# drowe67/radae

Hardware: AMD Instinct MI355X
Metric: vocoder-feature frames/sec (enc+chan+dec), model19 (higher is better)
Workload: dtype f32 I/O, 2xf16 (22-bit) MFMA operands, f32 accumulate (refine: f64 MFMA)

## Files before the change

### radae_amd/csrc/rade_core_step.hip

```cpp
#include <hip/hip_runtime.h>
#include <stdint.h>
#include <math.h>

#include "rade_devutil.h"

#define CS_THREADS 512
#define CS_WAVES (CS_THREADS / 64)
#define CS_PS 320
#define CS_WMAX 864

template <typename T> __device__ __forceinline__ T cs_gload(const T *p) { return *(const __attribute__((address_space(1))) T *)p; }

struct CsShared {
    __attribute__((aligned(16))) float x[CS_WMAX];
    __attribute__((aligned(16))) float hist[2][CS_WMAX];
    __attribute__((aligned(16))) float vin[96];
    __attribute__((aligned(16))) float h[5][96];
    __attribute__((aligned(16))) float hc[96];
    __attribute__((aligned(16))) float gh[288];
    __attribute__((aligned(16))) float pa[CS_WAVES][CS_PS];
    __attribute__((aligned(16))) float pb[CS_WAVES][CS_PS];
};

struct Rows3 { const float *r[3]; };
__device__ __forceinline__ const float *cs_in(const float *v, int) { return v; }
__device__ __forceinline__ const float *cs_in(const Rows3 &v, int q) { return v.r[q]; }
template <class T> __device__ __forceinline__ T *cs_prow(T (*part)[CS_PS], int w, int) { return part[w]; }
template <class T> __device__ __forceinline__ T *cs_prow(T (*part)[3][CS_PS], int w, int q) { return part[w][q]; }
template <int R> __device__ __forceinline__ int cs_wave()
{
    if constexpr (R == 3) return __builtin_amdgcn_readfirstlane((int)(threadIdx.x >> 6)); else return threadIdx.x >> 6;
}

template <int NRB, int NCI> struct WQ { f16x8 w[NRB][NCI]; };
template <int NRB, int NCI, int I0 = 0, int I1 = NCI>
__device__ __forceinline__ void cs_issue(const rd_mv &L, WQ<NRB, NCI> &r)
{
    const int lane = threadIdx.x & 63, wave = threadIdx.x >> 6, nch = L.K >> 3;
#pragma unroll
    for (int i = I0; i < I1; i++) {
        const int c = min(wave + CS_WAVES * i, nch - 1);
#pragma unroll
        for (int rb = 0; rb < NRB; rb++) r.w[rb][i] = cs_gload((const f16x8 *)(L.wq + ((size_t)c * (NRB * 64) + rb * 64 + lane) * 8));
    }
}
template <int NRB, int NCI>
__device__ __forceinline__ void cs_consume(const rd_mv &L, const WQ<NRB, NCI> &r, const float *v0, int K0, const float *v1, float (*part)[CS_PS])
{
    const int lane = threadIdx.x & 63, wave = threadIdx.x >> 6, nch = L.K >> 3;
    float acc[NRB];
#pragma unroll
    for (int rb = 0; rb < NRB; rb++) acc[rb] = 0.0f;
#pragma unroll
    for (int i = 0; i < NCI; i++) {
        const int c = wave + CS_WAVES * i, k = 8 * min(c, nch - 1);
        const float *src = k < K0 ? v0 + k : v1 + (k - K0);
        f32x4 a = *(const f32x4 *)src, b = *(const f32x4 *)(src + 4);
// ... 275 lines not shown
    cs_issue<2, CCI, C2, CCI>(a.conv[l], cq);
    if (!LAST) cs_issue<3, 1>(a.ghh[l + 1], hn);
    __builtin_amdgcn_sched_barrier(0);
    cs_acc3_range<2, CCI, C1, C2>(a.conv[l], cq, t0, cin, xr, cacc);
    __builtin_amdgcn_sched_barrier(0);
    cs_acc3_range<2, CCI, C2, CCI>(a.conv[l], cq, t0, cin, xr, cacc);
    cs_store3<2>(cacc, sh->pa);
    if (!LAST) cs_consume<3, 1>(a.ghh[l + 1], hn, sh->h[l + 1], H, sh->h[l + 1], sh->pb);
    __builtin_amdgcn_sched_barrier(0);
    if (!LAST) cs_issue<3, GNEXT, 0, (GNEXT < 6 ? GNEXT : 6)>(a.gin[l + 1], gnext);
    __syncthreads();
    if (tid < 96) {
#pragma unroll
        for (int q = 0; q < 3; q++) sh->x[q][cin + tid] = clamp1(tanhf(cs_row(a.conv[l], sh->pa, tid, q)));
    } else if (!LAST && tid >= 128 && tid < 128 + 3 * H) sh->gh[tid - 128] = cs_row(a.ghh[l + 1], sh->pb, tid - 128);
    __syncthreads();
}

__global__ __launch_bounds__(CS_THREADS) void k_tx_frame3(const rd_core_args *ap, unsigned seq)
{
    extern __shared__ __attribute__((aligned(16))) unsigned char cs_raw[];
    CsShared3 *sh = (CsShared3 *)cs_raw;
    const rd_core_args &a = *ap;
    const int tid = threadIdx.x, W = 864, H = 64;
    WQ<3, 1> g0, h0;
    cs_issue<3, 1>(a.gin[0], g0); cs_issue<3, 1>(a.ghh[0], h0);
    for (int i = tid; i < 2 * W; i += CS_THREADS) sh->hist[i / W][i % W] = a.hist[i];
    if (tid < 5 * H) sh->h[tid / H][tid % H] = a.h[tid];
    if (tid < 3 * 96) { const int q = tid / 96, c = tid % 96; sh->vin[q][c] = c < a.n_in ? a.in[q * a.n_in + c] : 0.0f; }
    __syncthreads();
    const Rows3 vr = { { sh->vin[0], sh->vin[1], sh->vin[2] } };
    cs_f32_product<2, 3>(a.dense1, 1, vr, sh->pa);
    cs_consume<3, 1>(a.ghh[0], h0, sh->h[0], H, sh->h[0], sh->pb);
    __syncthreads();
    if (tid < 64) {
#pragma unroll
        for (int q = 0; q < 3; q++) sh->x[q][tid] = clamp1(tanhf(cs_row(a.dense1, sh->pa, tid, q)));
    } else if (tid >= 128 && tid < 128 + 3 * H) sh->gh[tid - 128] = cs_row(a.ghh[0], sh->pb, tid - 128);
    __syncthreads();
    WQ<3, 4> g1; WQ<3, 6> g2; WQ<3, 9> g3; WQ<3, 11> g4;
    cs_enc_layer3<1, 4, 4, false>(sh, a, 0, 64, g0, g1);
    cs_enc_layer3<4, 9, 6, false>(sh, a, 1, 224, g1, g2);
    cs_enc_layer3<6, 14, 9, false>(sh, a, 2, 384, g2, g3);
    cs_enc_layer3<9, 19, 11, false>(sh, a, 3, 544, g3, g4);
    cs_enc_layer3<11, 24, 11, true>(sh, a, 4, 704, g4, g4);
    const Rows3 xr = { { sh->x[0], sh->x[1], sh->x[2] } };
    cs_f32_product<14, 3>(a.out, 2, xr, sh->pa);
    for (int i = tid; i < W; i += CS_THREADS) { a.hist[i] = sh->x[2][i]; a.hist[W + i] = sh->x[1][i]; }
    if (tid < 5 * H) a.h[tid] = sh->h[tid / H][tid % H];
    __syncthreads();
    if (tid < 3 * RD_LATENT) { const int q = tid / RD_LATENT, c = tid % RD_LATENT; sh->zs[q * RD_LATENT + c] = cs_row(a.out, sh->pa, c, q); }
    __syncthreads();
    const float *zs = sh->zs;
    const rd_tables *tab = ap->tab;
    float2 *out = (float2 *)ap->iq_out;
    if (tid < RD_M) {
        f32x2 acc[RD_NS + 1];
#pragma unroll
        for (int s = 0; s <= RD_NS; s++) acc[s] = (f32x2){ 0.0f, 0.0f };
#pragma unroll 6
        for (int c = 0; c < RD_NC; c++) {
            const float2 w = ld2(tab->Winv[c], tid);
            acc[0] = idft_term(acc[0], make_float2(tab->P[c] * tab->pilot_gain, 0.0f * tab->pilot_gain), w);
#pragma unroll
            for (int s = 1; s <= RD_NS; s++) { const int k = (s - 1) * RD_NC + c; acc[s] = idft_term(acc[s], make_float2(zs[2 * k], zs[2 * k + 1]), w); }
        }
#pragma unroll
        for (int s = 0; s <= RD_NS; s++) {
            const float2 v = pa_limit(make_float2(acc[s][0], acc[s][1]));
            out[s * RD_SYM + RD_NCP + tid] = v;
            if (tid >= RD_M - RD_NCP) out[s * RD_SYM + tid - (RD_M - RD_NCP)] = v;
        }
        __threadfence_system();
    }
    __syncthreads();
    if (tid == 0 && ap->done) { __threadfence_system(); *(volatile unsigned *)ap->done = seq; }
}
extern "C" int rd_launch_tx_frame(const rd_core_args *a_dev, unsigned seq, rd_stream_t s)
{
    rd_dyn_lds_once<k_tx_frame3, (int)sizeof(CsShared3)>();
    hipLaunchKernelGGL(k_tx_frame3, dim3(1), dim3(CS_THREADS), sizeof(CsShared3), (hipStream_t)s, a_dev, seq);
    return (int)hipGetLastError();
}

extern "C" int rd_launch_core_step(const rd_core_args *a, rd_stream_t s)
{
    if (a->is_enc) rd_dyn_lds_once<k_core_enc_step, (int)sizeof(CsShared)>(); else rd_dyn_lds_once<k_core_dec_step, (int)sizeof(CsShared)>();
    if (a->is_enc) hipLaunchKernelGGL(k_core_enc_step, dim3(1), dim3(CS_THREADS), sizeof(CsShared), (hipStream_t)s, *a);
    else hipLaunchKernelGGL(k_core_dec_step, dim3(1), dim3(CS_THREADS), sizeof(CsShared), (hipStream_t)s, *a);
    return (int)hipGetLastError();
}
```

### radae_amd/csrc/rade_dev.h

```cpp
#ifndef RADE_DEV_H
#define RADE_DEV_H

#include <stdint.h>

#ifdef __cplusplus
extern "C" {
#endif

#define RD_M        160
#define RD_NCP      32
#define RD_SYM      192
#define RD_NC       30
#define RD_NS       4
#define RD_NMF      960
#define RD_NEOO     1152
#define RD_RXBUF    2112
#define RD_NFC      40
#define RD_NQ       16
#define RD_NTAP     101
#define RD_NINMAX   1120
#define RD_LATENT   80
#define RD_ZMF      240
#define RD_FEAT_MF  432
#define RD_NEOOBITS 180
#define RD_ENC_W    864
#define RD_DEC_W    736
#define RD_ENC_IN   96
#define RD_RX_ROUND_MAX 128
#define RD_DEC_ROWS_MAX (3 * RD_RX_ROUND_MAX)

typedef struct {
    float Winv[RD_NC][RD_M][2];
    float Wfwd[RD_M][RD_NC][2];
    float P[RD_NC], Pend[RD_NC];
    float p[RD_M][2], pend[RD_M][2];
    float eoo[RD_NEOO][2];
    float Pmat[RD_NC][2][3][2];
    float eq_rot[RD_NC][2];
    float bpf_h[RD_NTAP + 3];
    float bpf_E[RD_NEOO][2];
    float p_w[RD_M][RD_NFC][2];
    double fcoarse[RD_NFC];
    float pilot_gain;
    float snr_c1, snr_c2;
    float pad;
} rd_tables;

typedef struct {
    int mem_len;
    int grid_off;
    float phase[2];
    float mem[102][2];
} rd_bpf_state;

typedef struct {
    int state, nin, tmax, tmax_candidate, valid_count, uw_errors, synced_count, mf;
    int f_ind_max, dec_reset_pending, n_out_frames, pad0;
    uint32_t lcg; int has_eoo, dt_valid;
    int pad1;
    double fmax, foff_err, rx_phase[2];
    double rx_theta;
    double Dthresh, Dtmax12, Dtmax12_eoo;
    float snr_est, pad2[3];
    unsigned rxmax[4];
    long long consumed;
    rd_bpf_state bpf;
    float rx_buf[RD_RXBUF][2];
    float rowsum1[RD_NMF], rowsum2[RD_NMF];
} rd_rx_stream;

typedef struct {
    int n_calls;
    int n_rows;
    int uw_from_row;
    int consumed;
    int row_reset[RD_DEC_ROWS_MAX];
    int call_ret[RD_RX_ROUND_MAX];
    int call_row_lo[RD_RX_ROUND_MAX], call_row_hi[RD_RX_ROUND_MAX];
    int call_trace_idx[RD_RX_ROUND_MAX];
    int out_base;
    int pad[3];
} rd_rx_round;

typedef struct {
    int state_before, state_after, nin_before, nin_after, ret, tmax, f_ind_max, valid_count;
    int uw_errors, synced_count, snr_int, pad;
    double fmax, Dthresh, Dtmax12, Dtmax12_eoo;
    float snrdB_3k_est; float pad2;
} rd_rx_trace;

typedef void *rd_stream_t;

typedef struct {
    const float *a1; long a1_sb, a1_st; int K1;
    const float *a0; long a0_sb, a0_st; int K0;
    const int *reset; int reset_sb;
    const int *n_rows;
    const float *Wp; const float *bias;
    const unsigned short *Wp16;
    const float *Wscale;
    float *y; long y_sb, y_st; int N;
    int B, T, act;
} rd_gemm_args;
int rd_launch_gemm(const rd_gemm_args *a, rd_stream_t s);
long rd_pack_weights(const float *W, int N, int K, float *out);
long rd_packed_size(int N, int K);

typedef struct {
    const float *gi; long gi_sb, gi_st;
    const float *Whh; const float *bhh;
    float *h;
    float *out; long out_sb, out_st;
    const int *reset; int reset_sb;
    const int *n_rows;
    int B, T, H;
    unsigned short *outf; int outf_NQ, outf_col;
} rd_scan_args;
int rd_launch_gru_scan(const rd_scan_args *a, rd_stream_t s);

#define RD_EF_KB   (RD_ENC_W / 16)
#define RD_EF_TILE (RD_EF_KB * 1024)
typedef struct {
    const unsigned short *xf; int NQ;
    int B, T, K0, K1, dil;
    const unsigned short *Wp16; const float *Wscale; const float *bias; int N, act;
    float *y; long y_sb, y_st;
    unsigned short *yf; int ycol;
    int seq_taps, no_pair;
    int pair;
    const float *xin; int Kin; const float *Wp;
} rd_encf_args;
int rd_launch_encf_gemm(const rd_encf_args *a, rd_stream_t s);
int rd_launch_encf_dense1(const rd_encf_args *a, rd_stream_t s);
int rd_launch_encf_hist(unsigned short *xf, int NQ, float *x32, long x32_sb, int B, int T, int dir, rd_stream_t s);

int rd_launch_enc_pack(const float *features, float *xin, int B, int T, rd_stream_t s);
int rd_launch_pad_rows(const float *src, float *dst, long R, int K, int Kpad, rd_stream_t s);
int rd_launch_chan_symbol(const float *z, const float *H, const float *noise, float *out, long n_real, int mode, float p0, float p1, unsigned long long seed, rd_stream_t s);
int rd_launch_carry_rows(float *x, int B, int Tcap, int W, int nhist, int T, const int *n_rows, rd_stream_t s);
int rd_launch_ofdm_mod(const rd_tables *tab, const float *z, void *tx, long tx_stride, int B, int n_mf, int linear, rd_stream_t s);
int rd_launch_ofdm_mod_mp(const rd_tables *tab, const float *z, void *tx, long tx_stride, int B, int n_mf, const void *G, void *mp, double *part, int linear, rd_stream_t s);
int rd_launch_eoo_build(const rd_tables *tab, const float *bits, float *eoo, int B, rd_stream_t s);
int rd_launch_copy_eoo(const float *eoo, void *out, long stride, int B, rd_stream_t s);

enum { RD_IRX_LS = 0, RD_IRX_MEAN6 = 1, RD_IRX_ALL = 2, RD_IRX_NONE = 3 };
typedef struct {
    const rd_tables *tab; const void *rx; long rx_stride;
    const float *foff;
    int n_mf, time_offset, eq, coarse_mag, B;
    float mag_scale;
    float *z_hat;
    double *part;
    const float *z_ref; long long *n_err;
} rd_irx_args;
int rd_launch_irx(const rd_irx_args *a, rd_stream_t s);

#define RD_LOSS_WG 64
typedef struct {
    const float *feat; long f_stride; int f_row;
    const float *hat; long h_stride; int h_row;
    const int *len;
    double *part_v; int *part_s; int n_blk;
    double *loss; int *start;
    float *frame_loss; long fl_stride; int max_hat;
    int B;
} rd_loss_args;
int rd_launch_loss(const rd_loss_args *a, rd_stream_t s);

#define RD_RS_NCH 8
typedef struct {
    const rd_tables *tab; const float *z, *H; const void *noise; float *z_hat;
    int B, n_steps, has_phase; float sigma, ph_re, ph_im;
    const float *sigma_b;
    unsigned long long seed;
    double *part;
    double *stats;
} rd_rs_args;
int rd_launch_rs_pa(const rd_rs_args *a, rd_stream_t s);

#define RD_CLK_TILE 1024
#define RD_CLK_PHASES 256
#define RD_CLK_TAPS 32
typedef struct { long long step_q, t0_q, n0, in_base; int n_in, n_out; } rd_clk_stream;
typedef struct {
    const void *x; long x_stride; void *y; long y_stride;
    const rd_clk_stream *ps;
    const float *taps;
    int mode, B, max_out;
} rd_clk_args;
int rd_launch_clk_resample(const rd_clk_args *a, rd_stream_t s);

#define RD_WIRE_NCH_MAX 64
// ... 339 lines not shown
```

### radae_amd/csrc/rade_engine.c

```c
#define _GNU_SOURCE

#include <pthread.h>
#include <time.h>
#include <sched.h>
#include <stdio.h>
#include <stdlib.h>
#include <string.h>
#include <stdint.h>
#include <math.h>

#include "rade_batch.h"
#include "rade_api.h"
#include "rade_host.h"
#include "rade_engine.h"

#define CHK(x) do { hipError_t e_ = (x); if (e_ != hipSuccess) { fprintf(stderr, "rade: HIP error %s at %s:%d\n", hipGetErrorString(e_), __FILE__, __LINE__); goto fail; } } while (0)

static int g_engines_open;
double rade_host_cpu_quota(void)
{
    cpu_set_t set; double n = 1.0;
    if (sched_getaffinity(0, sizeof set, &set) == 0) n = (double)CPU_COUNT(&set);
    FILE *f = fopen("/sys/fs/cgroup/cpu.max", "r");
    if (f) {
// ... 141 lines not shown
    }
    if (tx) {
        h->enc_hist_frag = 0;
        if (h->tx_bpf) hipMemcpyAsync(h->tx_bpf, h->tx_bpf_init, sizeof(rd_bpf_state) * h->B, hipMemcpyDeviceToDevice, st);
        r.enc_h = h->enc_h[0];
        r.enc_x = h->enc_x; r.enc_x_sb = (long)(2 + h->Tcap) * RD_ENC_W;
    }
    rd_launch_reset(&r, st);
}

void rade_batch_rx_reset(rade_batch *h) { ON_DEV(h); reset_on(h, 0, 1, NULL); hipDeviceSynchronize(); }

void rade_batch_reset(rade_batch *h, void *stream) { ON_DEV(h); reset_on(h, 1, 1, stream); }

void rade_batch_rx_set_lcg(rade_batch *h, const unsigned *seeds_host)
{
    ON_DEV(h);
    if (!h) return;
    for (int b = 0; b < h->B; b++) h->lcg_seeds[b] = seeds_host ? seeds_host[b] : 1u;
    hipMemcpy(h->d_lcg_seeds, h->lcg_seeds, sizeof(unsigned) * h->B, hipMemcpyHostToDevice);
    rade_batch_rx_reset(h);
}

void rade_batch_tx_reset(rade_batch *h) { ON_DEV(h); reset_on(h, 1, 0, NULL); hipDeviceSynchronize(); }

rade_batch *rade_batch_open_mem(const void *blob, size_t blob_len, const rade_batch_config *cfg)
{
    rade_batch *h = NULL;
    rd_model m; int have_model = 0;
    if (!cfg || cfg->n_streams <= 0 || cfg->max_tx_mf <= 0) { fprintf(stderr, "rade: bad batch config\n"); return NULL; }
    int ndev = 0;
    if (hipGetDeviceCount(&ndev) != hipSuccess || ndev <= 0) {
        fprintf(stderr, "rade: no HIP device available -- this library has no CPU fallback\n");
        return NULL;
    }
    CHK(hipSetDevice(cfg->device));
    if (rd_model_parse(blob, blob_len, &m)) return NULL;
    have_model = 1;
    h = calloc(1, sizeof *h);
    if (!h) { rd_model_free(&m); return NULL; }
    __atomic_add_fetch(&g_engines_open, 1, __ATOMIC_RELAXED);
    h->B = cfg->n_streams; h->max_tx_mf = cfg->max_tx_mf; h->device = cfg->device; h->flags = cfg->flags;
    h->trace_cap = cfg->rx_trace_calls; h->Tcap = 3 * cfg->max_tx_mf;
    h->unsync_off_after = cfg->disable_unsync != 0.0f ? (int)((double)cfg->disable_unsync * 8000.0 / RD_NMF) : -1;
    const size_t B = (size_t)h->B, T = (size_t)h->Tcap;
    h->R = getenv("RADE_ROUND_CALLS") ? atoi(getenv("RADE_ROUND_CALLS")) : RD_RX_ROUND_MAX;
    if (h->R < 1) h->R = 1;
    if (h->R > RD_RX_ROUND_MAX) h->R = RD_RX_ROUND_MAX;
    h->dec_rows = getenv("RADE_DEC_ROWS") ? atoi(getenv("RADE_DEC_ROWS")) : 48;
    if (h->dec_rows < 3) h->dec_rows = 3;
    if (h->dec_rows > 63) h->dec_rows = 63;
    const size_t DR = (size_t)h->dec_rows;

    rd_tables *tab = malloc(sizeof *tab);
    rd_tables_fill(tab);
    h->d_tab = dev_upload(h, tab, sizeof *tab);
    h->corrq16 = upload_table16(h, tab, rd_corrq16_table_fill, RD_CORRQ16_HALFS);
    h->corra16 = upload_table16(h, tab, rd_corra16_table_fill, RD_CORRA16_HALFS);
    h->wfwd16 = upload_table16(h, tab, rd_wfwd16_table_fill, RD_WFWD16_HALFS);
    h->bpf16 = upload_table16(h, tab, rd_bpf16_table_fill, RD_BPF16_HALFS);
    free(tab);
    {
        double vm[8][RD_M];
        for (int n = 0; n < RD_M; n++) { const double nu = ((double)n - 79.5) / 80.0; double v = 1.0; for (int m = 0; m < 8; m++) { vm[m][n] = v; v *= nu; } }
        h->vm = dev_upload(h, vm, sizeof vm);
    }
    h->rx_lds = rd_rx_sync_prepare();
    h->rx_census = getenv("RADE_RX2_CENSUS") ? atoi(getenv("RADE_RX2_CENSUS")) : 0;
    if (h->alloc_failed || h->rx_lds <= 0) goto fail;

    int err = 0;
    h->feat_in = m.enc_dense1.n_in; h->enc_kpad = (h->feat_in + 15) & ~15; h->bottleneck1 = (cfg->flags & RADE_BATCH_BOTTLENECK1) != 0;
    err |= upload_lin(h, &h->enc_dense1, m.enc_dense1.w, m.enc_dense1.b, NULL, 64, h->feat_in, h->enc_kpad);
    err |= upload_lin(h, &h->enc_zdense, m.enc_zdense.w, m.enc_zdense.b, NULL, 80, 864, 864);
    err |= upload_lin(h, &h->dec_dense1, m.dec_dense1.w, m.dec_dense1.b, NULL, 96, 80, 80);
    err |= upload_lin(h, &h->dec_output, m.dec_output.w, m.dec_output.b, NULL, h->feat_in, 736, 736);
    for (int l = 0; l < 5 && !err; l++) {
        err |= upload_lin(h, &h->enc_gin[l], m.enc_gru[l].w_ih, m.enc_gru[l].b_ih, m.enc_gru[l].s_ih, 192, ENC_IN[l], ENC_IN[l]);
        err |= upload_lin(h, &h->dec_gin[l], m.dec_gru[l].w_ih, m.dec_gru[l].b_ih, m.dec_gru[l].s_ih, 288, DEC_IN[l], DEC_IN[l]);
        err |= upload_lin(h, &h->enc_conv[l], m.enc_conv[l].w, m.enc_conv[l].b, m.enc_conv[l].row_scale, 96, m.enc_conv[l].n_in, m.enc_conv[l].n_in);
        err |= upload_lin(h, &h->dec_conv[l], m.dec_conv[l].w, m.dec_conv[l].b, m.dec_conv[l].row_scale, 32, m.dec_conv[l].n_in, m.dec_conv[l].n_in);
        err |= upload_lin(h, &h->dec_glu[l], m.dec_glu[l].w, NULL, m.dec_glu[l].row_scale, 96, 96, 96);
        h->enc_whh[l] = dev_upload(h, m.enc_gru[l].w_hh, sizeof(float) * 192 * 64);
        h->enc_bhh[l] = dev_upload(h, m.enc_gru[l].b_hh, sizeof(float) * 192);
        h->dec_whh[l] = dev_upload(h, m.dec_gru[l].w_hh, sizeof(float) * 288 * 96);
        h->dec_bhh[l] = dev_upload(h, m.dec_gru[l].b_hh, sizeof(float) * 288);
        if (m.dec_gru[l].s_hh) {
            unsigned short *pa = malloc(sizeof(unsigned short) * rd_packed16a_size(288, 96)); float *scl = malloc(sizeof(float) * 288);
            const long nq = (pa && scl) ? rd_pack_weights_q16_a16(m.dec_gru[l].w_hh, m.dec_gru[l].s_hh, 288, 96, pa, scl) : -1;
            if (nq > 0) { h->dec_whq[l] = dev_upload_opt(h, pa, sizeof(unsigned short) * nq); h->dec_whs[l] = dev_upload_opt(h, scl, sizeof(float) * 288); }
            free(pa); free(scl);
        }
    }
    if (err || h->alloc_failed) { fprintf(stderr, "rade: weight upload failed\n"); goto fail; }

    h->enc_xin = dev_zeros(h, sizeof(float) * B * T * RD_ENC_IN);
    h->enc_x = dev_zeros(h, sizeof(float) * B * (2 + T) * RD_ENC_W);
    h->enc_gi = dev_zeros(h, sizeof(float) * B * T * 192);
    h->enc_nq = 1 + (h->Tcap + 31) / 32;
    h->enc_seq_taps = getenv("RADE_ENCF_SEQ_TAPS") != NULL;
    h->enc_no_pair = getenv("RADE_ENCF_NO_PAIR") != NULL;
    if (B * T > 16384 && !getenv("RADE_ENC_ROWS")) {
        h->enc_xf = dev_alloc_opt(h, sizeof(unsigned short) * B * h->enc_nq * RD_EF_TILE, 1);
        if (!h->enc_xf && !getenv("RADE_VERBOSE_0"))
            fprintf(stderr, "rade: no device memory for the encoder's fragment buffer (%.1f MB): the float32-row kernels serve every call (slower encoder GEMMs, same results to the last bits documented in rade_batch.h)\n",
                    1e-6 * sizeof(unsigned short) * (double)B * h->enc_nq * RD_EF_TILE);
    }
    h->enc_z = dev_zeros(h, sizeof(float) * B * T * RD_LATENT);
    h->eoo = dev_zeros(h, sizeof(float) * B * RD_NEOO * 2);
    h->eoo_bits = dev_zeros(h, sizeof(float) * B * RD_NEOOBITS);
    h->bypass_dec = (cfg->flags & RADE_BATCH_BYPASS_DEC) != 0;
    h->tx_linear = (cfg->flags & RADE_BATCH_TX_LINEAR) != 0;
    if (h->tx_linear && (cfg->flags & RADE_BATCH_TX_BPF)) { fprintf(stderr, "rade: RADE_BATCH_TX_LINEAR cannot be combined with RADE_BATCH_TX_BPF (the filter clips)\n"); goto fail; }
    if (cfg->flags & RADE_BATCH_TX_BPF) {
// ... 679 lines not shown
```

### radae_amd/csrc/rade_host.c

```c
#include "rade_host.h"
#include "rade_batch.h"

#include <math.h>
#include <stdio.h>
#include <stdlib.h>
#include <string.h>

#define PI_D 3.14159265358979323846

static void pa_limit_host(float *re, float *im)
{
    float mag = hypotf(*re, *im), ang = atan2f(*im, *re), t = tanhf(mag);
    *re = t * cosf(ang); *im = t * sinf(ang);
}

void rd_tables_fill(rd_tables *T)
{
    static const float barker13[13] = { 1, 1, 1, 1, 1, -1, -1, 1, 1, -1, 1, -1, 1 };
    float w[RD_NC];
    memset(T, 0, sizeof *T);
    const float two_pi = (float)(2.0 * PI_D);
    for (int c = 0; c < RD_NC; c++) w[c] = (two_pi * (float)(15 + c)) / 160.0f;
    for (int c = 0; c < RD_NC; c++)
        for (int n = 0; n < RD_M; n++) {
// ... 430 lines not shown
                    o[0] = hi; o[64 * 8] = lo;
                }
}
void rd_corra16_table_fill(const rd_tables *T, unsigned short *out )
{
    static double q[RD_NQ][RD_M], alr[RD_NQ][RD_NFC], ali[RD_NQ][RD_NFC];
    corr_basis(T, q, alr, ali);
    for (int nt = 0; nt < 5; nt++)
        for (int lane = 0; lane < 64; lane++)
            for (int j = 0; j < 8; j++) {
                const int n = 16 * nt + (lane & 15), f = n >> 1, cpp = n & 1;
                const int g = lane >> 4, np_ = j < 4 ? 4 * g + j : 16 + 4 * g + (j - 4), r = np_ >> 1, cp = np_ & 1;
                const double ar = alr[r][f], ai = ali[r][f];
                const float v = (float)(1024.0 * (cpp == 0 ? (cp == 0 ? ar : -ai) : (cp == 0 ? ai : ar)));
                const unsigned short hi = f32_to_f16(v), lo = f32_to_f16(v - f16_to_f32(hi));
                unsigned short *o = out + (((size_t)nt * 2) * 64 + lane) * 8 + j;
                o[0] = hi; o[64 * 8] = lo;
            }
}
double rd_corr_tables_check(const rd_tables *T)
{
    static double q[RD_NQ][RD_M], alr[RD_NQ][RD_NFC], ali[RD_NQ][RD_NFC];
    corr_basis(T, q, alr, ali);
    double worst = 0.0;
    for (int m = 0; m < RD_M; m++)
        for (int f = 0; f < RD_NFC; f++) {
            double re = 0.0, im = 0.0;
            for (int r = 0; r < RD_NQ; r++) {
                const double sr = (double)T->p[m][0] * q[r][m], si = (double)T->p[m][1] * q[r][m];
                re += alr[r][f] * sr - ali[r][f] * si; im += alr[r][f] * si + ali[r][f] * sr;
            }
            const double d = hypot(re - (double)T->p_w[m][f][0], im - (double)T->p_w[m][f][1]);
            if (d > worst) worst = d;
        }
    return worst;
}

void rd_wfwd16_table_fill(const rd_tables *T, unsigned short *out )
{
    for (int tile = 0; tile < 2; tile++)
        for (int s = 0; s < 10; s++)
            for (int lane = 0; lane < 64; lane++)
                for (int j = 0; j < 8; j++) {
                    const int c = 16 * tile + (lane & 15);
                    const int k = 32 * s + 8 * (lane >> 4) + j, n = k >> 1, comp = k & 1;
                    float v = 0.0f;
                    if (c < RD_NC) v = 4096.0f * (comp == 0 ? T->Wfwd[n][c][0] : -T->Wfwd[n][c][1]);
                    const unsigned short hi = f32_to_f16(v), lo = f32_to_f16(v - f16_to_f32(hi));
                    unsigned short *o = out + ((((size_t)tile * 10 + s) * 2) * 64 + lane) * 8 + j;
                    o[0] = hi; o[64 * 8] = lo;
                }
}

void rd_bpf16_table_fill(const rd_tables *T, unsigned short *out )
{
    for (int ks = 0; ks < 4; ks++)
        for (int lane = 0; lane < 64; lane++)
            for (int j = 0; j < 8; j++) {
                const int r = lane & 15, m = 32 * ks + 8 * (lane >> 4) + j, t = m - r;
                const float v = (t >= 0 && t < RD_NTAP) ? 1024.0f * T->bpf_h[t] : 0.0f;
                const unsigned short hi = f32_to_f16(v), lo = f32_to_f16(v - f16_to_f32(hi));
                unsigned short *o = out + (((size_t)ks * 2) * 64 + lane) * 8 + j;
                o[0] = hi; o[64 * 8] = lo;
            }
}

static double bessel_i0(double x)
{
    double s = 1.0, t = 1.0;
    for (int k = 1; k < 40; k++) { t *= (x * 0.5) / k; s += t * t; }
    return s;
}

void rade_resample_taps(float *out )
{
    const double i0b = bessel_i0(10.0);
    for (int p = 0; p <= 256; p++) {
        const double f = p / 256.0, sf = sin(PI_D * (p <= 128 ? f : 1.0 - f));
        double g[32], sum = 0.0;
        for (int j = 0; j < 32; j++) {
            const int k = j - 15;
            const double t = (double)k - f, u = t / 16.0;
            const double sinc = t == 0.0 ? 1.0 : ((k & 1) ? sf : -sf) / (PI_D * t);
            g[j] = fabs(t) <= 16.0 ? sinc * bessel_i0(10.0 * sqrt(1.0 - u * u)) / i0b : 0.0;
            sum += g[j];
        }
        for (int j = 0; j < 32; j++) out[p * 32 + j] = (float)(g[j] / sum);
    }
}

int rd_resample_q(double t0, double ppm, long long *step_q, long long *t0_q)
{
    if (!(fabs(ppm) <= 50000.0) || !(fabs(t0) <= 536870912.0)) return -1;
    *step_q = llrint((1.0 + ppm * 1e-6) * 4294967296.0);
    *t0_q = llrint(t0 * 4294967296.0);
    return 0;
}

long long rade_resample_count(long long in_end, double t0, double ppm)
{
    long long step_q, t0_q;
    if (rd_resample_q(t0, ppm, &step_q, &t0_q)) return -1;
    const __int128 need = ((__int128)in_end << 32) - t0_q;
    if (need <= 0) return 0;
    const __int128 n = (need + step_q - 1) / step_q;
    return n * step_q > ((__int128)1 << 62) ? -1 : (long long)n;
// ... 337 lines not shown
```

### radae_amd/csrc/rade_host.h

```cpp
#ifndef RADE_HOST_H
#define RADE_HOST_H

#include <stddef.h>

#include "rade_dev.h"
#include "rade_batch.h"

#ifdef __cplusplus
extern "C" {
#endif

typedef struct { int n_in, n_out; float *w, *b; float *row_scale; } rd_linear;
typedef struct { int n_in, hid; float *w_ih, *w_hh, *b_ih, *b_hh; float *s_ih, *s_hh; } rd_gru;

typedef struct {
    rd_linear enc_dense1, enc_zdense, dec_dense1, dec_output;
    rd_gru enc_gru[5], dec_gru[5];
    rd_linear enc_conv[5], dec_conv[5];
    rd_linear dec_glu[5];
} rd_model;

const char *rd_find_default_model(const char *hint, char *buf, size_t n);

void rd_tables_fill(rd_tables *T);
int rd_model_parse(const void *blob, size_t len, rd_model *m);
void rd_model_free(rd_model *m);

long rd_packed16_size(int N, int K);
#define RD_CORRQ16_HALFS (2 * 10 * 2 * 64 * 8)
#define RD_CORRA16_HALFS (5 * 2 * 64 * 8)
#define RD_WFWD16_HALFS  (2 * 10 * 2 * 64 * 8)
#define RD_BPF16_HALFS   (4 * 2 * 64 * 8)
void rd_corrq16_table_fill(const rd_tables *T, unsigned short *out);
void rd_corra16_table_fill(const rd_tables *T, unsigned short *out);
double rd_corr_tables_check(const rd_tables *T);
void rd_wfwd16_table_fill(const rd_tables *T, unsigned short *out);
void rd_bpf16_table_fill(const rd_tables *T, unsigned short *out);
long rd_pack_weights_f16x2(const float *W, int N, int K, unsigned short *out);
long rd_pack_weights_q16(const float *W, const float *row_scale, int N, int K, unsigned short *out, float *scale_out);
int rd_chunkmajor_q16(const float *W, const float *row_scale, int N, int K, int Kpad, int Npad, unsigned short *out);
void rd_chunkmajor_f32(const float *W, int N, int K, int Kpad, int Npad, float *out);
long rd_packed16a_size(int N, int K);
long rd_pack_weights_q16_a16(const float *W, const float *row_scale, int N, int K, unsigned short *out, float *scale_out);
long rd_pack_weights_f16x2_a16(const float *W, int N, int K, unsigned short *out);
int rd_resample_q(double t0, double ppm, long long *step_q, long long *t0_q);
int rd_rate_reduce(int L, int M, int *Lr, int *Mr, int *T);
void rd_cno_table(int N, float *out);
void rd_cno_finish(const rade_cno_plan_t *q, const rade_cno_params *p, const double *bands, int n_windows, rade_cno_result *res);
#ifdef __cplusplus
}
#endif
void *rd_core_tx_open(const void *blob, int len, const rd_tables *d_tab);
void rd_core_tx_close(void *t);
int rd_core_tx_frame(void *t, const float *features_in, float *tx_out);
struct rade_batch;
const rd_tables *rd_batch_tables(const struct rade_batch *h);
int rd_batch_has_tx_bpf(const struct rade_batch *h);

#endif
```

### radae_amd/csrc/rade_kernels.hip

```cpp
#include "rade_devutil.h"

__device__ float g_zero_row[2048];

#include "rade_gemm.h"
#include "rade_gru_scan.h"
#include "rade_rows.h"
#include "rade_ofdm_mod.h"
#include "rade_chan.h"
```

### radae_amd/csrc/rade_ofdm_mod.h

```cpp
template <bool LINEAR>
__global__ __launch_bounds__(192) void k_ofdm_mod(const rd_tables *tab, const float *z, float2 *tx, long tx_stride, int n_mf)
{
    __shared__ float2 sym[RD_NS + 1][RD_NC];
    const int mf = blockIdx.x, b = blockIdx.y, tid = threadIdx.x;
    const float *zf = z + ((size_t)b * n_mf + mf) * RD_ZMF;
    const float pg = LINEAR ? 1.0f : tab->pilot_gain;
    if (tid < RD_NC) sym[0][tid] = make_float2(tab->P[tid] * pg, 0.0f * pg);
    if (tid < 120) sym[1 + tid / RD_NC][tid % RD_NC] = make_float2(zf[2 * tid], zf[2 * tid + 1]);
    __syncthreads();
    float2 *out = tx + (size_t)b * tx_stride + (size_t)mf * RD_NMF;
    if (tid < RD_M) {
        f32x2 acc[RD_NS + 1];
#pragma unroll
        for (int s = 0; s <= RD_NS; s++) acc[s] = (f32x2){ 0.0f, 0.0f };
#pragma unroll 6
        for (int c = 0; c < RD_NC; c++) {
            const float2 w = ld2(tab->Winv[c], tid);
#pragma unroll
            for (int s = 0; s <= RD_NS; s++) acc[s] = idft_term(acc[s], sym[s][c], w);
        }
#pragma unroll
        for (int s = 0; s <= RD_NS; s++) {
            const float2 v = LINEAR ? make_float2(acc[s][0], acc[s][1]) : pa_limit(make_float2(acc[s][0], acc[s][1]));
            out[s * RD_SYM + RD_NCP + tid] = v;
            if (tid >= RD_M - RD_NCP) out[s * RD_SYM + tid - (RD_M - RD_NCP)] = v;
        }
    }
}
extern "C" int rd_launch_ofdm_mod(const rd_tables *tab, const float *z, void *tx, long tx_stride, int B, int n_mf, int linear, rd_stream_t s)
{
    if (B <= 0 || n_mf <= 0) return 0;
    if (linear) hipLaunchKernelGGL(k_ofdm_mod<true>, dim3(n_mf, B), dim3(192), 0, (hipStream_t)s, tab, z, (float2 *)tx, tx_stride, n_mf);
    else hipLaunchKernelGGL(k_ofdm_mod<false>, dim3(n_mf, B), dim3(192), 0, (hipStream_t)s, tab, z, (float2 *)tx, tx_stride, n_mf);
    return (int)hipGetLastError();
}

template <bool LINEAR>
__global__ __launch_bounds__(192) void k_ofdm_mod_mp(const rd_tables *tab, const float *z, float2 *tx, long tx_stride, int n_mf, const float2 *G, float2 *mp, double *part)
{
    __shared__ float2 sym[RD_NS + 1][RD_NC];
    __shared__ float2 prevsym[RD_NC];
    __shared__ float2 fr[16 + RD_NMF];
    __shared__ double red[2][4];
    const int mf = blockIdx.x, b = blockIdx.y, tid = threadIdx.x;
    const float *zf = z + ((size_t)b * n_mf + mf) * RD_ZMF;
    const float pg = LINEAR ? 1.0f : tab->pilot_gain;
    if (tid < RD_NC) sym[0][tid] = make_float2(tab->P[tid] * pg, 0.0f * pg);
    if (tid < 120) sym[1 + tid / RD_NC][tid % RD_NC] = make_float2(zf[2 * tid], zf[2 * tid + 1]);
    if (tid >= 128 && tid < 128 + RD_NC && mf > 0) { const int c = tid - 128; prevsym[c] = make_float2(zf[-RD_ZMF + 2 * (90 + c)], zf[-RD_ZMF + 2 * (90 + c) + 1]); }
    __syncthreads();
    if (tid < RD_M) {
        f32x2 acc[RD_NS + 1];
#pragma unroll
        for (int s = 0; s <= RD_NS; s++) acc[s] = (f32x2){ 0.0f, 0.0f };
#pragma unroll 6
        for (int c = 0; c < RD_NC; c++) {
            const float2 w = ld2(tab->Winv[c], tid);
#pragma unroll
            for (int s = 0; s <= RD_NS; s++) acc[s] = idft_term(acc[s], sym[s][c], w);
        }
#pragma unroll
        for (int s = 0; s <= RD_NS; s++) {
            const float2 v = LINEAR ? make_float2(acc[s][0], acc[s][1]) : pa_limit(make_float2(acc[s][0], acc[s][1]));
            fr[16 + s * RD_SYM + RD_NCP + tid] = v;
            if (tid >= RD_M - RD_NCP) fr[16 + s * RD_SYM + tid - (RD_M - RD_NCP)] = v;
        }
    } else if (tid < RD_M + 16) {
        const int n = RD_M - 16 + (tid - RD_M);
        float2 a = make_float2(0.0f, 0.0f);
        if (mf > 0) { f32x2 ac = { 0.0f, 0.0f }; for (int c = 0; c < RD_NC; c++) ac = idft_term(ac, prevsym[c], ld2(tab->Winv[c], n)); a = LINEAR ? make_float2(ac[0], ac[1]) : pa_limit(make_float2(ac[0], ac[1])); }
        fr[tid - RD_M] = a;
    }
    __syncthreads();
    const size_t base = (size_t)mf * RD_NMF;
    const f32x4 *Gb = (const f32x4 *)G + (size_t)b * n_mf * RD_NMF;
    float2 *mpo = mp + (size_t)b * n_mf * RD_NMF + base;
    float2 *txo = tx ? tx + (size_t)b * tx_stride + base : nullptr;
    __shared__ float2 c2[16 + RD_NMF];
    float2 a1[5];
#pragma unroll
    for (int q = 0; q < 5; q++) {
        const int i = tid + 192 * q;
        const f32x4 g = Gb[base + i];
        const float2 x = fr[16 + i];
        a1[q] = cmul(x, make_float2(g[0], g[1]));
        c2[16 + i] = cmul(x, make_float2(g[2], g[3]));
    }
    if (tid < 16) { float2 v = make_float2(0.0f, 0.0f); if (mf > 0) { const f32x4 g = Gb[base - 16 + tid]; v = cmul(fr[tid], make_float2(g[2], g[3])); } c2[tid] = v; }
    __syncthreads();
    double s0 = 0.0, s1 = 0.0;
#pragma unroll
    for (int q = 0; q < 5; q++) {
        const int i = tid + 192 * q;
        const float2 x = fr[16 + i];
        const float2 m = cadd(a1[q], c2[i]);
        mpo[i] = m;
        if (txo) txo[i] = x;
        const float ax = hypotf(x.x, x.y), am = hypotf(m.x, m.y);
        s0 += (double)(ax * ax); s1 += (double)(am * am);
    }
    s0 = wave_sum_f64(s0); s1 = wave_sum_f64(s1);
    if ((tid & 63) == 0) { red[0][tid >> 6] = s0; red[1][tid >> 6] = s1; }
    __syncthreads();
    if (tid == 0) { part[((size_t)b * n_mf + mf) * 2] = (red[0][0] + red[0][1]) + red[0][2]; part[((size_t)b * n_mf + mf) * 2 + 1] = (red[1][0] + red[1][1]) + red[1][2]; }
}
extern "C" int rd_launch_ofdm_mod_mp(const rd_tables *tab, const float *z, void *tx, long tx_stride, int B, int n_mf, const void *G, void *mp, double *part, int linear, rd_stream_t s)
{
    if (B <= 0 || n_mf <= 0) return 0;
    if (linear) hipLaunchKernelGGL(k_ofdm_mod_mp<true>, dim3(n_mf, B), dim3(192), 0, (hipStream_t)s, tab, z, (float2 *)tx, tx_stride, n_mf, (const float2 *)G, (float2 *)mp, part);
    else hipLaunchKernelGGL(k_ofdm_mod_mp<false>, dim3(n_mf, B), dim3(192), 0, (hipStream_t)s, tab, z, (float2 *)tx, tx_stride, n_mf, (const float2 *)G, (float2 *)mp, part);
    return (int)hipGetLastError();
}

__global__ __launch_bounds__(192) void k_eoo_build(const rd_tables *tab, const float *bits, float2 *eoo)
{
    __shared__ float2 sym[RD_NS - 1][RD_NC];
    const int b = blockIdx.x, tid = threadIdx.x;
    float2 *out = eoo + (size_t)b * RD_NEOO;
    for (int i = tid; i < RD_NEOO; i += blockDim.x) out[i] = ld2(tab->eoo, i);
    if (!bits) return;
    if (tid < 90) sym[tid / RD_NC][tid % RD_NC] = make_float2(bits[b * RD_NEOOBITS + 2 * tid], bits[b * RD_NEOOBITS + 2 * tid + 1]);
    __syncthreads();
    if (tid < RD_M) {
        for (int s = 0; s < RD_NS - 1; s++) {
            float2 acc = make_float2(0.0f, 0.0f);
            for (int c = 0; c < RD_NC; c++) acc = cadd(acc, cmul(sym[s][c], ld2(tab->Winv[c], tid)));
            const float2 v = pa_limit(make_float2(acc.x * tab->pilot_gain, acc.y * tab->pilot_gain));
            out[(2 + s) * RD_SYM + RD_NCP + tid] = v;
            if (tid >= RD_M - RD_NCP) out[(2 + s) * RD_SYM + tid - (RD_M - RD_NCP)] = v;
        }
    }
}
extern "C" int rd_launch_eoo_build(const rd_tables *tab, const float *bits, float *eoo, int B, rd_stream_t s)
{
    hipLaunchKernelGGL(k_eoo_build, dim3(B), dim3(192), 0, (hipStream_t)s, tab, bits, (float2 *)eoo);
    return (int)hipGetLastError();
}
__global__ void k_copy_eoo(const float2 *eoo, float2 *out, long stride)
{
    const int b = blockIdx.x;
    for (int i = threadIdx.x; i < RD_NEOO; i += blockDim.x) out[(size_t)b * stride + i] = eoo[(size_t)b * RD_NEOO + i];
// ... 7 lines not shown
```

Measured before the change: 86.01 million.

## Compute OFDM modulator IDFT with split-f16 MFMA and precomputed pilot symbol

Replaces the scalar per-thread complex IDFT over 30 carriers in the OFDM modulator kernels and the fused tx frame step with a 16x16x32 f16 MFMA formulation. Symbols are block-scaled and split into hi/lo f16 planes, and the Winv table is prepacked as hi/lo f16 fragments. The pilot symbol, which is constant, is now computed once at init into a device table instead of every frame. The aim is to cut ALU work and per-thread table loads. The cost is an emulated extra-precision path built from several MFMA products, DPP shuffles to reassemble complex outputs, and a larger device table layout.

```diff
diff --git a/radae_amd/csrc/rade_core_step.hip b/radae_amd/csrc/rade_core_step.hip
--- a/radae_amd/csrc/rade_core_step.hip
+++ b/radae_amd/csrc/rade_core_step.hip
@@ -3,6 +3,7 @@
 #include <math.h>
 
 #include "rade_devutil.h"
+#include "rade_idft_mfma.h"
 
 #define CS_THREADS 512
 #define CS_WAVES (CS_THREADS / 64)
@@ -384,25 +385,22 @@
     if (tid < 3 * RD_LATENT) { const int q = tid / RD_LATENT, c = tid % RD_LATENT; sh->zs[q * RD_LATENT + c] = cs_row(a.out, sh->pa, c, q); }
     __syncthreads();
     const float *zs = sh->zs;
-    const rd_tables *tab = ap->tab;
+    const rd_tables_dev *td = (const rd_tables_dev *)ap->tab;
     float2 *out = (float2 *)ap->iq_out;
-    if (tid < RD_M) {
-        f32x2 acc[RD_NS + 1];
-#pragma unroll
-        for (int s = 0; s <= RD_NS; s++) acc[s] = (f32x2){ 0.0f, 0.0f };
-#pragma unroll 6
-        for (int c = 0; c < RD_NC; c++) {
-            const float2 w = ld2(tab->Winv[c], tid);
-            acc[0] = idft_term(acc[0], make_float2(tab->P[c] * tab->pilot_gain, 0.0f * tab->pilot_gain), w);
-#pragma unroll
-            for (int s = 1; s <= RD_NS; s++) { const int k = (s - 1) * RD_NC + c; acc[s] = idft_term(acc[s], make_float2(zs[2 * k], zs[2 * k + 1]), w); }
-        }
-#pragma unroll
-        for (int s = 0; s <= RD_NS; s++) {
-            const float2 v = pa_limit(make_float2(acc[s][0], acc[s][1]));
-            out[s * RD_SYM + RD_NCP + tid] = v;
-            if (tid >= RD_M - RD_NCP) out[s * RD_SYM + tid - (RD_M - RD_NCP)] = v;
-        }
+    ModPlanes<4> *pl = (ModPlanes<4> *)&sh->pa[0][0][0];
+    static_assert(sizeof(ModPlanes<4>) <= sizeof(sh->pa), "operand planes inside the partial-sum area");
+    const int t2 = rx_tid();
+    if (t2 < 128) {
+        const int q = t2 >> 5, c = t2 & 31;
+        mod_stage_symbol(pl, q, c, c < RD_NC ? make_float2(zs[2 * (q * RD_NC + c)], zs[2 * (q * RD_NC + c) + 1]) : make_float2(0.0f, 0.0f), true);
+    }
+    __syncthreads();
+    if (t2 < RD_SYM) {
+        out[t2] = mod_pilot_sample<false>(td, t2);
+        idft_frame_mfma<4, false, false>(td, pl, t2, nullptr, [&](int s, int n, float2 v) {
+            out[s * RD_SYM + RD_NCP + n] = v;
+            if (n >= RD_M - RD_NCP) out[s * RD_SYM + n - (RD_M - RD_NCP)] = v;
+        });
         __threadfence_system();
     }
     __syncthreads();
diff --git a/radae_amd/csrc/rade_dev.h b/radae_amd/csrc/rade_dev.h
--- a/radae_amd/csrc/rade_dev.h
+++ b/radae_amd/csrc/rade_dev.h
@@ -46,6 +46,13 @@
     float pad;
 } rd_tables;
 
+#define RD_WINV16_HALFS (10 * 2 * 2 * 64 * 8)
+typedef struct {
+    rd_tables t;
+    unsigned short winv16[RD_WINV16_HALFS];
+    float pilot[2][RD_SYM][2];
+} rd_tables_dev;
+
 typedef struct {
     int mem_len;
     int grid_off;
@@ -138,6 +145,7 @@
 int rd_launch_pad_rows(const float *src, float *dst, long R, int K, int Kpad, rd_stream_t s);
 int rd_launch_chan_symbol(const float *z, const float *H, const float *noise, float *out, long n_real, int mode, float p0, float p1, unsigned long long seed, rd_stream_t s);
 int rd_launch_carry_rows(float *x, int B, int Tcap, int W, int nhist, int T, const int *n_rows, rd_stream_t s);
+int rd_launch_mod_pilot(rd_tables_dev *td, rd_stream_t s);
 int rd_launch_ofdm_mod(const rd_tables *tab, const float *z, void *tx, long tx_stride, int B, int n_mf, int linear, rd_stream_t s);
 int rd_launch_ofdm_mod_mp(const rd_tables *tab, const float *z, void *tx, long tx_stride, int B, int n_mf, const void *G, void *mp, double *part, int linear, rd_stream_t s);
 int rd_launch_eoo_build(const rd_tables *tab, const float *bits, float *eoo, int B, rd_stream_t s);
diff --git a/radae_amd/csrc/rade_engine.c b/radae_amd/csrc/rade_engine.c
--- a/radae_amd/csrc/rade_engine.c
+++ b/radae_amd/csrc/rade_engine.c
@@ -217,14 +217,18 @@
     if (h->dec_rows > 63) h->dec_rows = 63;
     const size_t DR = (size_t)h->dec_rows;
 
-    rd_tables *tab = malloc(sizeof *tab);
+    rd_tables_dev *tabd = calloc(1, sizeof *tabd);
+    if (!tabd) goto fail;
+    rd_tables *tab = &tabd->t;
     rd_tables_fill(tab);
-    h->d_tab = dev_upload(h, tab, sizeof *tab);
+    rd_winv16_table_fill(tab, tabd->winv16);
+    h->d_tab = dev_upload(h, tabd, sizeof *tabd);
+    if (!h->d_tab || rd_launch_mod_pilot((rd_tables_dev *)h->d_tab, NULL) || hipDeviceSynchronize() != hipSuccess) h->alloc_failed = 1;
     h->corrq16 = upload_table16(h, tab, rd_corrq16_table_fill, RD_CORRQ16_HALFS);
     h->corra16 = upload_table16(h, tab, rd_corra16_table_fill, RD_CORRA16_HALFS);
     h->wfwd16 = upload_table16(h, tab, rd_wfwd16_table_fill, RD_WFWD16_HALFS);
     h->bpf16 = upload_table16(h, tab, rd_bpf16_table_fill, RD_BPF16_HALFS);
-    free(tab);
+    free(tabd);
     {
         double vm[8][RD_M];
         for (int n = 0; n < RD_M; n++) { const double nu = ((double)n - 79.5) / 80.0; double v = 1.0; for (int m = 0; m < 8; m++) { vm[m][n] = v; v *= nu; } }
diff --git a/radae_amd/csrc/rade_host.c b/radae_amd/csrc/rade_host.c
--- a/radae_amd/csrc/rade_host.c
+++ b/radae_amd/csrc/rade_host.c
@@ -506,6 +506,22 @@
                 }
 }
 
+void rd_winv16_table_fill(const rd_tables *T, unsigned short *out )
+{
+    for (int tile = 0; tile < 10; tile++)
+        for (int ks = 0; ks < 2; ks++)
+            for (int lane = 0; lane < 64; lane++)
+                for (int j = 0; j < 8; j++) {
+                    const int n = 16 * tile + (lane & 15);
+                    const int k = 32 * ks + 8 * (lane >> 4) + j, c = k >> 1, comp = k & 1;
+                    float v = 0.0f;
+                    if (c < RD_NC) v = 4096.0f * (comp == 0 ? T->Winv[c][n][0] : -T->Winv[c][n][1]);
+                    const unsigned short hi = f32_to_f16(v), lo = f32_to_f16(v - f16_to_f32(hi));
+                    unsigned short *o = out + ((((size_t)tile * 2 + ks) * 2) * 64 + lane) * 8 + j;
+                    o[0] = hi; o[64 * 8] = lo;
+                }
+}
+
 void rd_bpf16_table_fill(const rd_tables *T, unsigned short *out )
 {
     for (int ks = 0; ks < 4; ks++)
diff --git a/radae_amd/csrc/rade_host.h b/radae_amd/csrc/rade_host.h
--- a/radae_amd/csrc/rade_host.h
+++ b/radae_amd/csrc/rade_host.h
@@ -36,6 +36,7 @@
 double rd_corr_tables_check(const rd_tables *T);
 void rd_wfwd16_table_fill(const rd_tables *T, unsigned short *out);
 void rd_bpf16_table_fill(const rd_tables *T, unsigned short *out);
+void rd_winv16_table_fill(const rd_tables *T, unsigned short *out);
 long rd_pack_weights_f16x2(const float *W, int N, int K, unsigned short *out);
 long rd_pack_weights_q16(const float *W, const float *row_scale, int N, int K, unsigned short *out, float *scale_out);
 int rd_chunkmajor_q16(const float *W, const float *row_scale, int N, int K, int Kpad, int Npad, unsigned short *out);
diff --git a/radae_amd/csrc/rade_idft_mfma.h b/radae_amd/csrc/rade_idft_mfma.h
--- /dev/null
+++ b/radae_amd/csrc/rade_idft_mfma.h
@@ -0,0 +1,99 @@
+#ifndef RADE_IDFT_MFMA_H
+#define RADE_IDFT_MFMA_H
+#include "rade_devutil.h"
+
+static_assert(offsetof(rd_tables_dev, winv16) % 16 == 0 && offsetof(rd_tables_dev, pilot) % 8 == 0, "operand fragments are 16-byte loads, samples 8-byte ones");
+
+template <int NQ> struct ModPlanes {
+    __attribute__((aligned(16))) unsigned h[NQ][32], l[NQ][32];
+    float unsc[NQ];
+};
+
+template <int NQ> __device__ __forceinline__ void mod_stage_symbol(ModPlanes<NQ> *pl, int q, int c, float2 v, bool store)
+{
+    float m = fmaxf(fabsf(v.x), fabsf(v.y));
+    m = fmaxf(m, quad_dpp<QUAD_XOR1>(m)); m = fmaxf(m, quad_dpp<QUAD_XOR2>(m)); m = fmaxf(m, quad_dpp<ROW_ROR4>(m)); m = fmaxf(m, quad_dpp<ROW_ROR8>(m));
+    const float r0 = __int_as_float(__builtin_amdgcn_readlane(__float_as_int(m), 0)), r1 = __int_as_float(__builtin_amdgcn_readlane(__float_as_int(m), 16));
+    const float r2 = __int_as_float(__builtin_amdgcn_readlane(__float_as_int(m), 32)), r3 = __int_as_float(__builtin_amdgcn_readlane(__float_as_int(m), 48));
+    m = (threadIdx.x & 32) ? fmaxf(r2, r3) : fmaxf(r0, r1);
+    const int eb = min(max((int)((__float_as_uint(m) >> 23) & 0xffu), 32), 222);
+    const float sc = __uint_as_float((unsigned)(127 + 7 - (eb - 127)) << 23);
+    const float xr = v.x * sc, xi = v.y * sc;
+    typedef _Float16 f16x2 __attribute__((ext_vector_type(2)));
+    const f16x2 h2 = __builtin_bit_cast(f16x2, __builtin_amdgcn_cvt_pkrtz(xr, xi));
+    const _Float16 lr = (_Float16)(xr - (float)h2[0]), li = (_Float16)(xi - (float)h2[1]);
+    if (store) {
+        pl->h[q][c] = __builtin_bit_cast(unsigned, h2);
+        pl->l[q][c] = (unsigned)__builtin_bit_cast(unsigned short, lr) | ((unsigned)__builtin_bit_cast(unsigned short, li) << 16);
+        if (c == 0) pl->unsc[q] = __uint_as_float((unsigned)(eb - 7 - 12) << 23);
+    }
+}
+
+struct ModTile { f16x8 h[2], l[2]; };
+__device__ __forceinline__ ModTile mod_load_tile(const rd_tables_dev *td, int tile, int lane)
+{
+    typedef const __attribute__((address_space(1))) f16x8 glb_f16x8_t;
+    const unsigned short *pt = td->winv16 + ((size_t)tile * 2 * 2 * 64 + lane) * 8;
+    ModTile t;
+#pragma unroll
+    for (int ks = 0; ks < 2; ks++) { t.h[ks] = *(glb_f16x8_t *)(pt + (size_t)(ks * 2) * 512); t.l[ks] = *(glb_f16x8_t *)(pt + (size_t)(ks * 2 + 1) * 512); }
+    return t;
+}
+
+template <int NQ, bool LINEAR, bool AHEAD, class Put>
+__device__ __forceinline__ void idft_frame_mfma(const rd_tables_dev *td, const ModPlanes<NQ> *pl, int tid, const ModTile *first, Put put)
+{
+    static_assert(NQ == 4 || NQ == 5, "four data symbols, and the previous frame's last");
+    const int wave = tid >> 6, lane = tid & 63, col = lane & 15, g = lane >> 4;
+    if (wave >= 3) return;
+    const int q = col < 8 ? col >> 1 : NQ - 1;
+    const unsigned im_var = (col & 1) ? 0xffffffffu : 0u;
+    auto turn = [&](unsigned v) { const unsigned t = (v >> 16) | (((v & 0xffffu) ^ 0x8000u) << 16); return (t & im_var) | (v & ~im_var); };
+    u32x4 bh[2], bl[2];
+#pragma unroll
+    for (int ks = 0; ks < 2; ks++) {
+        const u32x4 vh = *(const u32x4 *)&pl->h[q][16 * ks + 4 * g], vl = *(const u32x4 *)&pl->l[q][16 * ks + 4 * g];
+#pragma unroll
+        for (int j = 0; j < 4; j++) { bh[ks][j] = turn(vh[j]); bl[ks][j] = turn(vl[j]); }
+    }
+    const float unsc = pl->unsc[q];
+    const bool up = col >= 8, odd = col & 1;
+    const int s = 1 + ((col & 7) >> 1);
+    ModTile cur;
+    if (AHEAD) cur = *first;
+#pragma unroll 1
+    for (int tile = wave; tile < 10; tile += 3) {
+        ModTile nxt;
+        if (AHEAD) { nxt = cur; if (tile + 3 < 10) nxt = mod_load_tile(td, tile + 3, lane); }
+        else cur = mod_load_tile(td, tile, lane);
+        const f16x8 (&Ah)[2] = cur.h, (&Al)[2] = cur.l;
+        f32x4 a0 = { 0.0f, 0.0f, 0.0f, 0.0f }, a2 = a0;
+#pragma unroll
+        for (int ks = 0; ks < 2; ks++) {
+            a0 = __builtin_amdgcn_mfma_f32_16x16x32_f16(Al[ks], __builtin_bit_cast(f16x8, bl[ks]), a0, 0, 0, 0);
+            a0 = __builtin_amdgcn_mfma_f32_16x16x32_f16(Al[ks], __builtin_bit_cast(f16x8, bh[ks]), a0, 0, 0, 0);
+            a2 = __builtin_amdgcn_mfma_f32_16x16x32_f16(Ah[ks], __builtin_bit_cast(f16x8, bh[ks]), a2, 0, 0, 0);
+            a0 = __builtin_amdgcn_mfma_f32_16x16x32_f16(Ah[ks], __builtin_bit_cast(f16x8, bl[ks]), a0, 0, 0, 0);
+        }
+        const f32x4 r = (a0 + a2) * unsc;
+        if (NQ == 5 && tile == 9) {
+            float p[4];
+#pragma unroll
+            for (int rr = 0; rr < 4; rr++) p[rr] = quad_dpp<QUAD_XOR1>(r[rr]);
+            if (col == 8 || col == 9) {
+                const float2 x0 = odd ? make_float2(p[2], r[2]) : make_float2(r[0], p[0]), x1 = odd ? make_float2(p[3], r[3]) : make_float2(r[1], p[1]);
+                const int n = 16 * tile + 4 * g + 2 * (int)odd;
+                put(5, n, LINEAR ? x0 : pa_limit(x0)); put(5, n + 1, LINEAR ? x1 : pa_limit(x1));
+            }
+        }
+        const float q2 = quad_dpp<ROW_ROR8>(r[2]), q3 = quad_dpp<ROW_ROR8>(r[3]);
+        const float w0 = up ? q2 : r[0], w1 = up ? q3 : r[1];
+        const float got = quad_dpp<QUAD_XOR1>(odd ? w0 : w1);
+        const float2 x = odd ? make_float2(got, w1) : make_float2(w0, got);
+        put(s, 16 * tile + 4 * g + 2 * (int)up + (int)odd, LINEAR ? x : pa_limit(x));
+        if (AHEAD) cur = nxt;
+    }
+}
+
+template <bool LINEAR> __device__ __forceinline__ float2 mod_pilot_sample(const rd_tables_dev *td, int i) { return ld2(td->pilot[LINEAR ? 1 : 0], i); }
+#endif
diff --git a/radae_amd/csrc/rade_kernels.hip b/radae_amd/csrc/rade_kernels.hip
--- a/radae_amd/csrc/rade_kernels.hip
+++ b/radae_amd/csrc/rade_kernels.hip
@@ -5,5 +5,6 @@
 #include "rade_gemm.h"
 #include "rade_gru_scan.h"
 #include "rade_rows.h"
+#include "rade_idft_mfma.h"
 #include "rade_ofdm_mod.h"
 #include "rade_chan.h"
diff --git a/radae_amd/csrc/rade_ofdm_mod.h b/radae_amd/csrc/rade_ofdm_mod.h
--- a/radae_amd/csrc/rade_ofdm_mod.h
+++ b/radae_amd/csrc/rade_ofdm_mod.h
@@ -1,31 +1,47 @@
 template <bool LINEAR>
 __global__ __launch_bounds__(192) void k_ofdm_mod(const rd_tables *tab, const float *z, float2 *tx, long tx_stride, int n_mf)
 {
-    __shared__ float2 sym[RD_NS + 1][RD_NC];
+    __shared__ ModPlanes<4> pl;
+    const rd_tables_dev *td = (const rd_tables_dev *)tab;
     const int mf = blockIdx.x, b = blockIdx.y, tid = threadIdx.x;
     const float *zf = z + ((size_t)b * n_mf + mf) * RD_ZMF;
-    const float pg = LINEAR ? 1.0f : tab->pilot_gain;
-    if (tid < RD_NC) sym[0][tid] = make_float2(tab->P[tid] * pg, 0.0f * pg);
-    if (tid < 120) sym[1 + tid / RD_NC][tid % RD_NC] = make_float2(zf[2 * tid], zf[2 * tid + 1]);
+    if (tid < 128) {
+        const int q = tid >> 5, c = tid & 31;
+        mod_stage_symbol(&pl, q, c, c < RD_NC ? make_float2(zf[2 * (q * RD_NC + c)], zf[2 * (q * RD_NC + c) + 1]) : make_float2(0.0f, 0.0f), true);
+    }
     __syncthreads();
     float2 *out = tx + (size_t)b * tx_stride + (size_t)mf * RD_NMF;
-    if (tid < RD_M) {
-        f32x2 acc[RD_NS + 1];
-#pragma unroll
-        for (int s = 0; s <= RD_NS; s++) acc[s] = (f32x2){ 0.0f, 0.0f };
-#pragma unroll 6
-        for (int c = 0; c < RD_NC; c++) {
-            const float2 w = ld2(tab->Winv[c], tid);
-#pragma unroll
-            for (int s = 0; s <= RD_NS; s++) acc[s] = idft_term(acc[s], sym[s][c], w);
+    out[tid] = mod_pilot_sample<LINEAR>(td, tid);
+    idft_frame_mfma<4, LINEAR, false>(td, &pl, tid, nullptr, [&](int s, int n, float2 v) {
+        out[s * RD_SYM + RD_NCP + n] = v;
+        if (n >= RD_M - RD_NCP) out[s * RD_SYM + n - (RD_M - RD_NCP)] = v;
+    });
+}
+__global__ __launch_bounds__(192) void k_mod_pilot(rd_tables_dev *td)
+{
+    __shared__ ModPlanes<4> pl;
+    const int tid = threadIdx.x;
+    for (int lin = 0; lin < 2; lin++) {
+        const float pg = lin ? 1.0f : td->t.pilot_gain;
+        if (tid < 128) {
+            const int q = tid >> 5, c = tid & 31;
+            mod_stage_symbol(&pl, q, c, (q == 0 && c < RD_NC) ? make_float2(td->t.P[c] * pg, 0.0f * pg) : make_float2(0.0f, 0.0f), true);
         }
-#pragma unroll
-        for (int s = 0; s <= RD_NS; s++) {
-            const float2 v = LINEAR ? make_float2(acc[s][0], acc[s][1]) : pa_limit(make_float2(acc[s][0], acc[s][1]));
-            out[s * RD_SYM + RD_NCP + tid] = v;
-            if (tid >= RD_M - RD_NCP) out[s * RD_SYM + tid - (RD_M - RD_NCP)] = v;
-        }
+        __syncthreads();
+        float2 *out = (float2 *)td->pilot[lin];
+        auto put = [&](int s, int n, float2 v) {
+            if (s != 1) return;
+            out[RD_NCP + n] = v;
+            if (n >= RD_M - RD_NCP) out[n - (RD_M - RD_NCP)] = v;
+        };
+        if (lin) idft_frame_mfma<4, true, false>(td, &pl, tid, nullptr, put); else idft_frame_mfma<4, false, false>(td, &pl, tid, nullptr, put);
+        __syncthreads();
     }
+}
+extern "C" int rd_launch_mod_pilot(rd_tables_dev *td, rd_stream_t s)
+{
+    hipLaunchKernelGGL(k_mod_pilot, dim3(1), dim3(192), 0, (hipStream_t)s, td);
+    return (int)hipGetLastError();
 }
 extern "C" int rd_launch_ofdm_mod(const rd_tables *tab, const float *z, void *tx, long tx_stride, int B, int n_mf, int linear, rd_stream_t s)
 {
@@ -38,39 +54,26 @@
 template <bool LINEAR>
 __global__ __launch_bounds__(192) void k_ofdm_mod_mp(const rd_tables *tab, const float *z, float2 *tx, long tx_stride, int n_mf, const float2 *G, float2 *mp, double *part)
 {
-    __shared__ float2 sym[RD_NS + 1][RD_NC];
-    __shared__ float2 prevsym[RD_NC];
+    __shared__ ModPlanes<5> pl;
     __shared__ float2 fr[16 + RD_NMF];
     __shared__ double red[2][4];
+    const rd_tables_dev *td = (const rd_tables_dev *)tab;
     const int mf = blockIdx.x, b = blockIdx.y, tid = threadIdx.x;
     const float *zf = z + ((size_t)b * n_mf + mf) * RD_ZMF;
-    const float pg = LINEAR ? 1.0f : tab->pilot_gain;
-    if (tid < RD_NC) sym[0][tid] = make_float2(tab->P[tid] * pg, 0.0f * pg);
-    if (tid < 120) sym[1 + tid / RD_NC][tid % RD_NC] = make_float2(zf[2 * tid], zf[2 * tid + 1]);
-    if (tid >= 128 && tid < 128 + RD_NC && mf > 0) { const int c = tid - 128; prevsym[c] = make_float2(zf[-RD_ZMF + 2 * (90 + c)], zf[-RD_ZMF + 2 * (90 + c) + 1]); }
+    {
+        const int q = tid >> 5, c = tid & 31;
+        const float *zq = tid < 128 ? zf + 2 * q * RD_NC : zf - RD_ZMF + 2 * 90;
+        const bool have = c < RD_NC && (tid < 128 || (q == 4 && mf > 0));
+        mod_stage_symbol(&pl, q, c, have ? make_float2(zq[2 * c], zq[2 * c + 1]) : make_float2(0.0f, 0.0f), q <= 4);
+    }
+    const ModTile first = mod_load_tile(td, min(tid >> 6, 2), tid & 63);
     __syncthreads();
-    if (tid < RD_M) {
-        f32x2 acc[RD_NS + 1];
-#pragma unroll
-        for (int s = 0; s <= RD_NS; s++) acc[s] = (f32x2){ 0.0f, 0.0f };
-#pragma unroll 6
-        for (int c = 0; c < RD_NC; c++) {
-            const float2 w = ld2(tab->Winv[c], tid);
-#pragma unroll
-            for (int s = 0; s <= RD_NS; s++) acc[s] = idft_term(acc[s], sym[s][c], w);
-        }
-#pragma unroll
-        for (int s = 0; s <= RD_NS; s++) {
-            const float2 v = LINEAR ? make_float2(acc[s][0], acc[s][1]) : pa_limit(make_float2(acc[s][0], acc[s][1]));
-            fr[16 + s * RD_SYM + RD_NCP + tid] = v;
-            if (tid >= RD_M - RD_NCP) fr[16 + s * RD_SYM + tid - (RD_M - RD_NCP)] = v;
-        }
-    } else if (tid < RD_M + 16) {
-        const int n = RD_M - 16 + (tid - RD_M);
-        float2 a = make_float2(0.0f, 0.0f);
-        if (mf > 0) { f32x2 ac = { 0.0f, 0.0f }; for (int c = 0; c < RD_NC; c++) ac = idft_term(ac, prevsym[c], ld2(tab->Winv[c], n)); a = LINEAR ? make_float2(ac[0], ac[1]) : pa_limit(make_float2(ac[0], ac[1])); }
-        fr[tid - RD_M] = a;
-    }
+    fr[16 + tid] = mod_pilot_sample<LINEAR>(td, tid);
+    idft_frame_mfma<5, LINEAR, true>(td, &pl, tid, &first, [&](int s, int n, float2 v) {
+        if (s == 5) { fr[n - (RD_M - 16)] = v; return; }
+        fr[16 + s * RD_SYM + RD_NCP + n] = v;
+        if (n >= RD_M - RD_NCP) fr[16 + s * RD_SYM + n - (RD_M - RD_NCP)] = v;
+    });
     __syncthreads();
     const size_t base = (size_t)mf * RD_NMF;
     const f32x4 *Gb = (const f32x4 *)G + (size_t)b * n_mf * RD_NMF;
@@ -86,7 +89,7 @@
         a1[q] = cmul(x, make_float2(g[0], g[1]));
         c2[16 + i] = cmul(x, make_float2(g[2], g[3]));
     }
-    if (tid < 16) { float2 v = make_float2(0.0f, 0.0f); if (mf > 0) { const f32x4 g = Gb[base - 16 + tid]; v = cmul(fr[tid], make_float2(g[2], g[3])); } c2[tid] = v; }
+    if (tid < 16) { float2 v = make_float2(0.0f, 0.0f); if (mf > 0) { const f32x4 gp = Gb[base - 16 + tid]; v = cmul(fr[tid], make_float2(gp[2], gp[3])); } c2[tid] = v; }
     __syncthreads();
     double s0 = 0.0, s1 = 0.0;
 #pragma unroll
```

Measured after the change: 86.39 million (median of 3 runs). About the same (+0.4%).
